# openai/Video-Pre-Training

Hardware: NVIDIA H100
Metric: frames/sec MinecraftPolicy fwd, 128x128x3 BxT=128x128 (higher is better)
Workload: dtype bf16

## Files before the change

video-pre-training_b200/csrc/common.cuh:

```cuda
#pragma once
#include <cuda.h>
#include <cuda_bf16.h>
#include <cuda_runtime.h>
#include <stdint.h>

#include "../../include/vpt_b200.h"

namespace vpt {

void set_error(const char* fmt, ...);
#define VPT_CHECK(cond, ...)                 \
    do {                                     \
        if (!(cond)) {                       \
            vpt::set_error(__VA_ARGS__);     \
            return VPT_ERR_ARG;              \
        }                                    \
    } while (0)
#define VPT_CUDA(expr)                                                                   \
    do {                                                                                 \
        cudaError_t _e = (expr);                                                         \
        if (_e != cudaSuccess) {                                                         \
            vpt::set_error("%s failed: %s (%s:%d)", #expr, cudaGetErrorString(_e), __FILE__, __LINE__); \
            return VPT_ERR_CUDA;                                                         \
        }                                                                                \
    } while (0)
#define VPT_LAUNCH_CHECK() VPT_CUDA(cudaGetLastError())
static int g_pdl = 0;
template <typename... KArgs, typename... Args>
static inline void launch_k(void (*kernel)(KArgs...), dim3 grid, dim3 block, size_t smem, cudaStream_t stream, Args&&... args) {
    cudaLaunchConfig_t cfg;
    memset(&cfg, 0, sizeof(cfg));
    cfg.gridDim = grid;
    cfg.blockDim = block;
    cfg.dynamicSmemBytes = smem;
    cfg.stream = stream;
    cudaLaunchAttribute attr[1];
    attr[0].id = cudaLaunchAttributeProgrammaticStreamSerialization;
    attr[0].val.programmaticStreamSerializationAllowed = 1;
    cfg.attrs = attr;
    cfg.numAttrs = g_pdl ? 1 : 0;
    (void)cudaLaunchKernelEx(&cfg, kernel, static_cast<KArgs>(args)...);
}


#ifndef VPT_NO_WATCHDOG
__device__ unsigned int g_device_error = 0;
#endif

__device__ __forceinline__ void pdl_sync() {
    asm volatile("griddepcontrol.launch_dependents;" ::: "memory");
    asm volatile("griddepcontrol.wait;" ::: "memory");
}
__device__ __forceinline__ uint32_t smem_u32(const void* p) { return (uint32_t)__cvta_generic_to_shared(p); }
__device__ __forceinline__ int lane_id() { return threadIdx.x & 31; }

__device__ __forceinline__ float warp_sum(float v) {
#pragma unroll
    for (int o = 16; o > 0; o >>= 1) v += __shfl_xor_sync(0xffffffffu, v, o);
    return v;
}
__device__ __forceinline__ float warp_max(float v) {
#pragma unroll
    for (int o = 16; o > 0; o >>= 1) v = fmaxf(v, __shfl_xor_sync(0xffffffffu, v, o));
    return v;
}

__device__ __forceinline__ uint32_t pack_bf16(float lo, float hi) {
    __nv_bfloat162 v = __floats2bfloat162_rn(lo, hi);
    return *reinterpret_cast<uint32_t*>(&v);
}
__device__ __forceinline__ float bf16_lo(uint32_t v) { return __uint_as_float(v << 16); }
__device__ __forceinline__ float bf16_hi(uint32_t v) { return __uint_as_float(v & 0xffff0000u); }
__device__ __forceinline__ float round_bf16(float v) { return __bfloat162float(__float2bfloat16_rn(v)); }

__device__ __forceinline__ void mbar_init(uint64_t* bar, uint32_t count) {
    asm volatile("mbarrier.init.shared::cta.b64 [%0], %1;" ::"r"(smem_u32(bar)), "r"(count));
}
__device__ __forceinline__ void fence_barrier_init() { asm volatile("fence.mbarrier_init.release.cluster;" ::: "memory"); }
__device__ __forceinline__ void fence_proxy_async() { asm volatile("fence.proxy.async.shared::cta;" ::: "memory"); }
__device__ __forceinline__ void mbar_expect_tx(uint64_t* bar, uint32_t bytes) {
    asm volatile("mbarrier.arrive.expect_tx.shared::cta.b64 _, [%0], %1;" ::"r"(smem_u32(bar)), "r"(bytes) : "memory");
}
__device__ __forceinline__ void mbar_arrive(uint64_t* bar) {
    asm volatile("mbarrier.arrive.shared::cta.b64 _, [%0];" ::"r"(smem_u32(bar)) : "memory");
}
__device__ __forceinline__ bool mbar_try_wait(uint64_t* bar, uint32_t parity) {
    uint32_t ok;
    asm volatile(
        "{\n\t.reg .pred p;\n\t"
        "mbarrier.try_wait.parity.shared::cta.b64 p, [%1], %2;\n\t"
        "selp.b32 %0, 1, 0, p;\n\t}"
        : "=r"(ok)
        : "r"(smem_u32(bar)), "r"(parity)
        : "memory");
    return ok != 0;
}
__device__ __forceinline__ bool mbar_try_wait_sleep(uint64_t* bar, uint32_t parity, uint32_t ns) {
    uint32_t ok;
    asm volatile(
        "{\n\t.reg .pred p;\n\t"
        "mbarrier.try_wait.parity.shared::cta.b64 p, [%1], %2, %3;\n\t"
        "selp.b32 %0, 1, 0, p;\n\t}"
        : "=r"(ok)
        : "r"(smem_u32(bar)), "r"(parity), "r"(ns)
        : "memory");
    return ok != 0;
}
__device__ __forceinline__ bool mbar_wait(uint64_t* bar, uint32_t parity, unsigned int code) {
    if (mbar_try_wait(bar, parity)) return true;
    const long long t0 = clock64();
    for (unsigned int it = 1;; ++it) {
        if (mbar_try_wait_sleep(bar, parity, 20000u)) return true;
        if ((it & 63u) == 0u) {
            if (*(volatile unsigned int*)&g_device_error != 0u) return false;
            if (clock64() - t0 > 3000000000LL) {
                atomicCAS(&g_device_error, 0u, code);
                return false;
            }
        }
    }
}

__device__ __forceinline__ void tma_prefetch_desc(const CUtensorMap* m) {
    asm volatile("prefetch.tensormap [%0];" ::"l"((uint64_t)m) : "memory");
}
__device__ __forceinline__ void tma_load_2d(void* dst, const CUtensorMap* m, uint64_t* bar, int c0, int c1) {
    asm volatile(
        "cp.async.bulk.tensor.2d.shared::cluster.global.tile.mbarrier::complete_tx::bytes [%0], [%1, {%3, %4}], [%2];" ::"r"(
            smem_u32(dst)),
        "l"((uint64_t)m), "r"(smem_u32(bar)), "r"(c0), "r"(c1)
        : "memory");
}
__device__ __forceinline__ void tma_load_4d(void* dst, const CUtensorMap* m, uint64_t* bar, int c0, int c1, int c2, int c3) {
    asm volatile(
        "cp.async.bulk.tensor.4d.shared::cluster.global.tile.mbarrier::complete_tx::bytes [%0], [%1, {%3, %4, %5, %6}], [%2];" ::"r"(
            smem_u32(dst)),
        "l"((uint64_t)m), "r"(smem_u32(bar)), "r"(c0), "r"(c1), "r"(c2), "r"(c3)
        : "memory");
}

__device__ __forceinline__ void tma_store_2d(const CUtensorMap* m, const void* src, int c0, int c1) {
    asm volatile("cp.async.bulk.tensor.2d.global.shared::cta.bulk_group [%0, {%2, %3}], [%1];" ::"l"((uint64_t)m), "r"(smem_u32(src)), "r"(c0),
                 "r"(c1)
                 : "memory");
}
__device__ __forceinline__ void bulk_commit() { asm volatile("cp.async.bulk.commit_group;" ::: "memory"); }
template <int N>
__device__ __forceinline__ void bulk_wait_read() {
    asm volatile("cp.async.bulk.wait_group.read %0;" ::"n"(N) : "memory");
}
template <int N>
__device__ __forceinline__ void bulk_wait_all() {
    asm volatile("cp.async.bulk.wait_group %0;" ::"n"(N) : "memory");
}
__device__ __forceinline__ void named_bar_sync(int id, int nthreads) { asm volatile("bar.sync %0, %1;" ::"r"(id), "r"(nthreads) : "memory"); }
__device__ __forceinline__ void named_bar_arrive(int id, int nthreads) { asm volatile("bar.arrive %0, %1;" ::"r"(id), "r"(nthreads) : "memory"); }

__device__ __forceinline__ void tma_load_2d_mc(void* dst, const CUtensorMap* m, uint64_t* bar, int c0, int c1, uint16_t cta_mask) {
    asm volatile(
        "cp.async.bulk.tensor.2d.shared::cluster.global.tile.mbarrier::complete_tx::bytes.multicast::cluster [%0], [%1, {%3, %4}], [%2], %5;" ::"r"(
            smem_u32(dst)),
        "l"((uint64_t)m), "r"(smem_u32(bar)), "r"(c0), "r"(c1), "h"(cta_mask)
        : "memory");
}

__device__ __forceinline__ void mbar_arrive_cluster(uint64_t* bar, uint32_t rank) {
    asm volatile(
        "{\n\t.reg .b32 ra;\n\t"
        "mapa.shared::cluster.u32 ra, %0, %1;\n\t"
        "mbarrier.arrive.release.cluster.shared::cluster.b64 _, [ra];\n\t}" ::"r"(smem_u32(bar)),
        "r"(rank)
        : "memory");
}
__device__ __forceinline__ uint32_t cluster_ctarank() {
    uint32_t r;
    asm volatile("mov.u32 %0, %%cluster_ctarank;" : "=r"(r));
    return r;
}
__device__ __forceinline__ void cluster_sync_all() {
    asm volatile("barrier.cluster.arrive.release.aligned;\n\tbarrier.cluster.wait.acquire.aligned;" ::: "memory");
}

__device__ __forceinline__ void wgmma_fence() { asm volatile("wgmma.fence.sync.aligned;" ::: "memory"); }
__device__ __forceinline__ void wgmma_commit() { asm volatile("wgmma.commit_group.sync.aligned;" ::: "memory"); }
template <int N>
__device__ __forceinline__ void wgmma_wait() { asm volatile("wgmma.wait_group.sync.aligned %0;" ::"n"(N) : "memory"); }
template <int N>
__device__ __forceinline__ void wgmma_reg_fence(float (&d)[N]) {
#pragma unroll
    for (int i = 0; i < N; ++i) asm volatile("" : "+f"(d[i])::"memory");
}

template <int TA, int TB>
__device__ __forceinline__ void wgmma_n64(float (&d)[32], uint64_t a_desc, uint64_t b_desc, uint32_t accumulate) {
    asm volatile(
        "{\n\t.reg .pred p;\n\t"
        "setp.ne.b32 p, %34, 0;\n\t"
        "wgmma.mma_async.sync.aligned.m64n64k16.f32.bf16.bf16 "
        "{%0, %1, %2, %3, %4, %5, %6, %7, %8, %9, %10, %11, %12, %13, %14, %15, %16, %17, %18, %19, %20, %21, %22, %23, %24, %25, %26, %27, %28, %29, %30, %31}, %32, %33, p, 1, 1, %35, %36;\n\t}"
        : "+f"(d[0]), "+f"(d[1]), "+f"(d[2]), "+f"(d[3]), "+f"(d[4]), "+f"(d[5]), "+f"(d[6]), "+f"(d[7]), "+f"(d[8]), "+f"(d[9]), "+f"(d[10]), "+f"(d[11]), "+f"(d[12]), "+f"(d[13]), "+f"(d[14]), "+f"(d[15]), "+f"(d[16]), "+f"(d[17]), "+f"(d[18]), "+f"(d[19]), "+f"(d[20]), "+f"(d[21]), "+f"(d[22]), "+f"(d[23]), "+f"(d[24]), "+f"(d[25]), "+f"(d[26]), "+f"(d[27]), "+f"(d[28]), "+f"(d[29]), "+f"(d[30]), "+f"(d[31])
        : "l"(a_desc), "l"(b_desc), "r"(accumulate), "n"(TA), "n"(TB)
        : "memory");
}

template <int TA, int TB>
__device__ __forceinline__ void wgmma_n128(float (&d)[64], uint64_t a_desc, uint64_t b_desc, uint32_t accumulate) {
    asm volatile(
        "{\n\t.reg .pred p;\n\t"
        "setp.ne.b32 p, %66, 0;\n\t"
        "wgmma.mma_async.sync.aligned.m64n128k16.f32.bf16.bf16 "
        "{%0, %1, %2, %3, %4, %5, %6, %7, %8, %9, %10, %11, %12, %13, %14, %15, %16, %17, %18, %19, %20, %21, %22, %23, %24, %25, %26, %27, %28, %29, %30, %31, %32, %33, %34, %35, %36, %37, %38, %39, %40, %41, %42, %43, %44, %45, %46, %47, %48, %49, %50, %51, %52, %53, %54, %55, %56, %57, %58, %59, %60, %61, %62, %63}, %64, %65, p, 1, 1, %67, %68;\n\t}"
        : "+f"(d[0]), "+f"(d[1]), "+f"(d[2]), "+f"(d[3]), "+f"(d[4]), "+f"(d[5]), "+f"(d[6]), "+f"(d[7]), "+f"(d[8]), "+f"(d[9]), "+f"(d[10]), "+f"(d[11]), "+f"(d[12]), "+f"(d[13]), "+f"(d[14]), "+f"(d[15]), "+f"(d[16]), "+f"(d[17]), "+f"(d[18]), "+f"(d[19]), "+f"(d[20]), "+f"(d[21]), "+f"(d[22]), "+f"(d[23]), "+f"(d[24]), "+f"(d[25]), "+f"(d[26]), "+f"(d[27]), "+f"(d[28]), "+f"(d[29]), "+f"(d[30]), "+f"(d[31]), "+f"(d[32]), "+f"(d[33]), "+f"(d[34]), "+f"(d[35]), "+f"(d[36]), "+f"(d[37]), "+f"(d[38]), "+f"(d[39]), "+f"(d[40]), "+f"(d[41]), "+f"(d[42]), "+f"(d[43]), "+f"(d[44]), "+f"(d[45]), "+f"(d[46]), "+f"(d[47]), "+f"(d[48]), "+f"(d[49]), "+f"(d[50]), "+f"(d[51]), "+f"(d[52]), "+f"(d[53]), "+f"(d[54]), "+f"(d[55]), "+f"(d[56]), "+f"(d[57]), "+f"(d[58]), "+f"(d[59]), "+f"(d[60]), "+f"(d[61]), "+f"(d[62]), "+f"(d[63])
        : "l"(a_desc), "l"(b_desc), "r"(accumulate), "n"(TA), "n"(TB)
        : "memory");
}

template <int R>
__device__ __forceinline__ void setmaxnreg_dec() { asm volatile("setmaxnreg.dec.sync.aligned.u32 %0;" ::"n"(R)); }
template <int R>
__device__ __forceinline__ void setmaxnreg_inc() { asm volatile("setmaxnreg.inc.sync.aligned.u32 %0;" ::"n"(R)); }

__device__ __forceinline__ uint64_t gmma_desc_sw128(uint32_t smem_addr, uint32_t lbo_bytes = 16u, uint32_t sbo_bytes = 1024u) {
    uint64_t d = 0;
    d |= (uint64_t)((smem_addr & 0x3FFFFu) >> 4);
    d |= (uint64_t)(lbo_bytes >> 4) << 16;
    d |= (uint64_t)(sbo_bytes >> 4) << 32;
    d |= (uint64_t)1 << 62;
    return d;
}

template <int NR>
__device__ __forceinline__ void wgmma_frag_store(const float (&d)[NR], float* stg, int pitch, int col0) {
    const int w = (threadIdx.x >> 5) & 3, l = threadIdx.x & 31;
    const int r0 = 16 * w + (l >> 2), c0 = col0 + 2 * (l & 3);
#pragma unroll
    for (int i = 0; i < NR / 4; ++i) {
        *reinterpret_cast<float2*>(stg + (size_t)r0 * pitch + c0 + 8 * i) = make_float2(d[4 * i], d[4 * i + 1]);
        *reinterpret_cast<float2*>(stg + (size_t)(r0 + 8) * pitch + c0 + 8 * i) = make_float2(d[4 * i + 2], d[4 * i + 3]);
    }
}
template <int C, int NR>
__device__ __forceinline__ void wgmma_frag_store_chunk(const float (&d)[NR], float* blk, int pitch) {
    static_assert(16 * C + 16 <= NR, "chunk outside the fragment");
    const int l = threadIdx.x & 31;
    float* dst = blk + (size_t)(l >> 2) * pitch + 2 * (l & 3);
#pragma unroll
    for (int i = 0; i < 4; ++i) {
        *reinterpret_cast<float2*>(dst + 8 * i) = make_float2(d[16 * C + 4 * i], d[16 * C + 4 * i + 1]);
        *reinterpret_cast<float2*>(dst + (size_t)8 * pitch + 8 * i) = make_float2(d[16 * C + 4 * i + 2], d[16 * C + 4 * i + 3]);
    }
}
__device__ __forceinline__ void stg_ld_32(const float* src, uint32_t (&v)[32]) {
#pragma unroll
    for (int q = 0; q < 8; ++q) {
        const float4 x = reinterpret_cast<const float4*>(src)[q];
        v[4 * q] = __float_as_uint(x.x); v[4 * q + 1] = __float_as_uint(x.y); v[4 * q + 2] = __float_as_uint(x.z); v[4 * q + 3] = __float_as_uint(x.w);
    }
}

}
```

video-pre-training_b200/csrc/firstconv.cuh:

```cuda
#pragma once
#include <type_traits>

#include "attention.cuh"
#include "common.cuh"

namespace vpt {

constexpr int kFcTile = 8;
constexpr int kFcConv = 2 * kFcTile + 1;
constexpr int kFcIn = kFcConv + 2;
constexpr int kFcThreads = 256;
constexpr int kFcPos = kFcConv * kFcConv;
constexpr int kFcMTiles = (kFcPos + 15) / 16;
constexpr int kFcPatchElems = kFcIn * kFcIn * 3;
constexpr int kFcPatchBytes = 2192;

template <typename TIN>
struct FcIn {
    static constexpr bool kF32 = std::is_same<TIN, float>::value;
    static constexpr int kKSteps = kF32 ? 6 : 4;
    static constexpr int kBPitch = 16 * kKSteps + 8;
    static constexpr int kPatches = kF32 ? 2 : 1;
};

template <bool F32OUT, typename TIN>
__global__ void __launch_bounds__(kFcThreads, 2) firstconv_pool_kernel(const TIN* __restrict__ img, const float* __restrict__ w,
                                                                       const float* __restrict__ bias, void* __restrict__ out_,
                                                                       float2* __restrict__ stat_part, int H, int W, int C0, long long total_tiles, int zp) {
    pdl_sync();
    extern __shared__ __align__(16) uint8_t fc_smem[];
    using In = FcIn<TIN>;
    constexpr int kBPitch = In::kBPitch, kKCols = 16 * In::kKSteps;
    __nv_bfloat16* patch = reinterpret_cast<__nv_bfloat16*>(fc_smem);
    __nv_bfloat16* patch_lo = reinterpret_cast<__nv_bfloat16*>(fc_smem + kFcPatchBytes);
    __nv_bfloat16* Bs = reinterpret_cast<__nv_bfloat16*>(fc_smem + In::kPatches * kFcPatchBytes);
    using CT = typename std::conditional<F32OUT, float, __nv_bfloat16>::type;
    const int CB = F32OUT ? 64 : C0;
    const int cpitch = CB + 8;
    CT* ctile = reinterpret_cast<CT*>(Bs + (size_t)C0 * kBPitch);
    CT* const out = reinterpret_cast<CT*>(out_);
    const int tiles_x = (W / 2) / kFcTile, tiles_y = (H / 2) / kFcTile;
    const int tiles = tiles_x * tiles_y;

    for (int i = threadIdx.x; i < C0 * kKCols; i += kFcThreads) {
        const int n = i / kKCols, k = i % kKCols;
        float v = 0.f;
        if (k >= 64) {
            if (k < 64 + 27) v = __ldg(w + n * 27 + k - 64);
        } else if (k < 27) {
            v = __ldg(w + n * 27 + k);
        } else if (k < 54) {
            const float x = __ldg(w + n * 27 + k - 27);
            v = x - __bfloat162float(__float2bfloat16_rn(x));
        } else if (k == 54) {
            v = __ldg(bias + n);
        } else if (k == 55) {
            const float x = __ldg(bias + n);
            v = x - __bfloat162float(__float2bfloat16_rn(x));
        }
        Bs[n * kBPitch + k] = __float2bfloat16_rn(v);
    }

    const int warp = threadIdx.x >> 5, lane = threadIdx.x & 31, g = lane >> 2, tg = lane & 3;
    int koff[4][4];
    bool kval[4][4];
#pragma unroll
    for (int s = 0; s < 4; ++s)
#pragma unroll
        for (int e = 0; e < 4; ++e) {
            const int k = 16 * s + 2 * tg + (e & 1) + ((e >> 1) << 3);
            const int kk = k < 27 ? k : k - 27;
            kval[s][e] = k < 54;
            koff[s][e] = kval[s][e] ? (kk / 9) * (kFcIn * 3) + kk % 9 : 0;
        }

    constexpr int kPE = (kFcPatchElems + kFcThreads - 1) / kFcThreads;
    int pe_row[kPE], pe_col[kPE];
#pragma unroll
    for (int j = 0; j < kPE; ++j) {
        const int i = threadIdx.x + j * kFcThreads;
        pe_row[j] = i / (kFcIn * 3);
        pe_col[j] = i % (kFcIn * 3);
    }
    TIN pre[kPE];
    auto prefetch = [&](long long tid) {
        const long long f = tid / tiles;
        const int tile = (int)(tid % tiles);
        const int Yin0 = 2 * (tile / tiles_x) * kFcTile - 2, Xin0 = 2 * (tile % tiles_x) * kFcTile - 2;
        const TIN* fimg = img + f * (long long)H * W * 3;
#pragma unroll
        for (int j = 0; j < kPE; ++j) {
            const int Y = Yin0 + pe_row[j], xb = Xin0 * 3 + pe_col[j];
            const bool ok = (threadIdx.x + j * kFcThreads < kFcPatchElems) && Y >= 0 && Y < H && xb >= 0 && xb < W * 3;
            pre[j] = ok ? __ldg(fimg + (long long)Y * W * 3 + xb) : (TIN)0;
        }
    };
    if ((long long)blockIdx.x < total_tiles) prefetch(blockIdx.x);

  for (long long tid = blockIdx.x; tid < total_tiles; tid += gridDim.x) {
    const long long f = tid / tiles;
    const int tile = (int)(tid % tiles);
    const int PY0 = (tile / tiles_x) * kFcTile, PX0 = (tile % tiles_x) * kFcTile;
    int any_lo = 0;
    if constexpr (In::kF32) {
        int nz = 0;
#pragma unroll
        for (int j = 0; j < kPE; ++j) {
            const int i = threadIdx.x + j * kFcThreads;
            if (i < kFcPatchElems) {
                const __nv_bfloat16 hi = __float2bfloat16_rn(pre[j]);
                const float lo = pre[j] - __bfloat162float(hi);
                patch[i] = hi;
                patch_lo[i] = __float2bfloat16_rn(lo);
                nz |= lo != 0.f;
            }
        }
        any_lo = __syncthreads_or(nz);
    } else {
#pragma unroll
        for (int j = 0; j < kPE; ++j) {
            const int i = threadIdx.x + j * kFcThreads;
            if (i < kFcPatchElems) patch[i] = __float2bfloat16_rn((float)pre[j]);
        }
    }
    if (tid + gridDim.x < total_tiles) prefetch(tid + gridDim.x);
    const int Ho = H / 2, Wo = W / 2, opitch = Wo + zp;
    CT* fout = out + f * (long long)(Ho + zp) * opitch * C0;
  for (int cg = 0; cg < C0; cg += CB) {
    __syncthreads();

    for (int mt = warp; mt < kFcMTiles; mt += kFcThreads / 32) {
        int pos[2], pbase[2];
        bool inimg[2];
#pragma unroll
        for (int rr = 0; rr < 2; ++rr) {
            const int p = min(mt * 16 + g + rr * 8, kFcPos - 1);
            pos[rr] = mt * 16 + g + rr * 8;
            const int cy = p / kFcConv, cx = p % kFcConv;
            pbase[rr] = (cy * kFcIn + cx) * 3;
            const int Y = 2 * PY0 - 1 + cy, X = 2 * PX0 - 1 + cx;
            inimg[rr] = (Y >= 0 && Y < H && X >= 0 && X < W);
        }
        uint32_t af[4][4];
#pragma unroll
        for (int s = 0; s < 4; ++s) {
#pragma unroll
            for (int rr = 0; rr < 2; ++rr) {
#pragma unroll
                for (int hh = 0; hh < 2; ++hh) {
                    const uint16_t lo = kval[s][2 * hh] ? *reinterpret_cast<const uint16_t*>(patch + pbase[rr] + koff[s][2 * hh]) : (uint16_t)0;
                    const uint16_t hi = kval[s][2 * hh + 1] ? *reinterpret_cast<const uint16_t*>(patch + pbase[rr] + koff[s][2 * hh + 1]) : (uint16_t)0;
                    af[s][rr + 2 * hh] = (uint32_t)lo | ((uint32_t)hi << 16);
                }
            }
        }
        if (tg == 3) af[3][0] = af[3][1] = 0x3F803F80u;

        for (int nh = cg / 64; nh < (cg + CB) / 64; ++nh) {
            float acc[8][4];
#pragma unroll
            for (int nt = 0; nt < 8; ++nt) acc[nt][0] = acc[nt][1] = acc[nt][2] = acc[nt][3] = 0.f;
#pragma unroll
            for (int s = 0; s < 4; ++s) {
#pragma unroll
                for (int np = 0; np < 4; ++np) {
                    uint32_t b0, b1, b2, b3;
                    const int nrow = nh * 64 + np * 16 + (lane & 7) + ((lane >> 4) << 3);
                    const int kcol = s * 16 + (((lane >> 3) & 1) << 3);
                    ldsm_x4(smem_u32(Bs + nrow * kBPitch + kcol), b0, b1, b2, b3);
                    mma_bf16_16816(acc[2 * np], af[s][0], af[s][1], af[s][2], af[s][3], b0, b1);
                    mma_bf16_16816(acc[2 * np + 1], af[s][0], af[s][1], af[s][2], af[s][3], b2, b3);
                }
            }
            if constexpr (In::kF32) {
                if (any_lo) {
#pragma unroll
                    for (int s = 0; s < 2; ++s) {
                        uint32_t af_lo[4];
#pragma unroll
                        for (int rr = 0; rr < 2; ++rr)
#pragma unroll
                            for (int hh = 0; hh < 2; ++hh) {
                                const int k = 16 * s + 2 * tg + 8 * hh;
                                const uint16_t lo = k < 27 ? *reinterpret_cast<const uint16_t*>(patch_lo + pbase[rr] + koff[s][2 * hh]) : (uint16_t)0;
                                const uint16_t hi = k + 1 < 27 ? *reinterpret_cast<const uint16_t*>(patch_lo + pbase[rr] + koff[s][2 * hh + 1]) : (uint16_t)0;
                                af_lo[rr + 2 * hh] = (uint32_t)lo | ((uint32_t)hi << 16);
                            }
#pragma unroll
                        for (int np = 0; np < 4; ++np) {
                            uint32_t b0, b1, b2, b3;
                            const int nrow = nh * 64 + np * 16 + (lane & 7) + ((lane >> 4) << 3);
                            const int kcol = 64 + s * 16 + (((lane >> 3) & 1) << 3);
                            ldsm_x4(smem_u32(Bs + nrow * kBPitch + kcol), b0, b1, b2, b3);
                            mma_bf16_16816(acc[2 * np], af_lo[0], af_lo[1], af_lo[2], af_lo[3], b0, b1);
                            mma_bf16_16816(acc[2 * np + 1], af_lo[0], af_lo[1], af_lo[2], af_lo[3], b2, b3);
                        }
                    }
                }
            }
#pragma unroll
            for (int rr = 0; rr < 2; ++rr) {
                if (pos[rr] >= kFcPos) continue;
                CT* crow = ctile + (size_t)pos[rr] * cpitch + (nh * 64 - cg) + 2 * tg;
#pragma unroll
                for (int nt = 0; nt < 8; ++nt) {
                    const float v0 = inimg[rr] ? acc[nt][2 * rr] : 0.f;
                    const float v1 = inimg[rr] ? acc[nt][2 * rr + 1] : 0.f;
                    if constexpr (F32OUT) *reinterpret_cast<float2*>(crow + nt * 8) = make_float2(v0, v1);
                    else *reinterpret_cast<uint32_t*>(crow + nt * 8) = pack_bf16(v0, v1);
                }
            }
        }
    }
    __syncthreads();

    if constexpr (F32OUT) {
        const int C4 = CB / 4;
        for (int i = threadIdx.x; i < kFcTile * kFcTile * C4; i += kFcThreads) {
            const int c4 = i % C4, px = (i / C4) % kFcTile, py = i / (C4 * kFcTile);
            float4 m = make_float4(0.f, 0.f, 0.f, 0.f);
#pragma unroll
            for (int dy = 0; dy < 3; ++dy)
#pragma unroll
                for (int dx = 0; dx < 3; ++dx) {
                    const int p = (2 * py + dy) * kFcConv + 2 * px + dx;
                    const float4 v = *reinterpret_cast<const float4*>(ctile + (size_t)p * cpitch + 4 * c4);
                    m.x = fmaxf(m.x, v.x); m.y = fmaxf(m.y, v.y); m.z = fmaxf(m.z, v.z); m.w = fmaxf(m.w, v.w);
                }
            *reinterpret_cast<float4*>(fout + ((long long)(PY0 + py) * opitch + PX0 + px) * C0 + cg + 4 * c4) = m;
        }
    } else {
    const int C8 = C0 / 8;
    for (int i = threadIdx.x; i < kFcTile * kFcTile * C8; i += kFcThreads) {
        const int c8 = i % C8, px = (i / C8) % kFcTile, py = i / (C8 * kFcTile);
        uint4 m = make_uint4(0, 0, 0, 0);
#pragma unroll
        for (int dy = 0; dy < 3; ++dy)
#pragma unroll
            for (int dx = 0; dx < 3; ++dx) {
                const int p = (2 * py + dy) * kFcConv + 2 * px + dx;
                const uint4 v = *reinterpret_cast<const uint4*>(ctile + (size_t)p * cpitch + 8 * c8);
                m.x = bf16x2_max(m.x, v.x); m.y = bf16x2_max(m.y, v.y);
                m.z = bf16x2_max(m.z, v.z); m.w = bf16x2_max(m.w, v.w);
            }
        *reinterpret_cast<uint4*>(fout + ((long long)(PY0 + py) * opitch + PX0 + px) * C0 + 8 * c8) = m;
    }
    }
  }
    if (zp) {
        const int C8 = C0 * (int)sizeof(CT) / 16;
        uint4* fo = reinterpret_cast<uint4*>(fout);
        const bool right = (PX0 + kFcTile == Wo), bottom = (PY0 + kFcTile == Ho);
        if (right)
            for (int i = threadIdx.x; i < kFcTile * C8; i += kFcThreads)
                fo[((long long)(PY0 + i / C8) * opitch + Wo) * C8 + (i % C8)] = make_uint4(0, 0, 0, 0);
        if (bottom)
            for (int i = threadIdx.x; i < (kFcTile + (right ? 1 : 0)) * C8; i += kFcThreads)
                fo[((long long)Ho * opitch + PX0 + i / C8) * C8 + (i % C8)] = make_uint4(0, 0, 0, 0);
    }
    __syncthreads();
    if (stat_part) {
        for (int c = threadIdx.x; c < C0; c += kFcThreads) {
            float cs = 0.f, css = 0.f;
            for (int py = 0; py < kFcTile; ++py)
                for (int px = 0; px < kFcTile; ++px) {
                    const CT o = fout[((long long)(PY0 + py) * opitch + PX0 + px) * C0 + c];
                    float v;
                    if constexpr (F32OUT) v = o;
                    else v = __bfloat162float(o);
                    cs += v;
                    css = fmaf(v, v, css);
                }
            stat_part[(f * tiles + tile) * C0 + c] = make_float2(cs, css);
        }
    }
  }
}

}

extern "C" int vpt_firstconv_stat_parts(int32_t F, int32_t H, int32_t W, int32_t C0) {
    (void)F;
    return (H / 16) * (W / 16) * C0;
}

extern "C" int vpt_set_firstconv_mode(int32_t mode) {
    (void)mode;
    return VPT_OK;
}

namespace vpt {

template <typename TIN>
static int firstconv_pool_launch(const char* fn, const TIN* img, const float* w, const float* bias, void* out, float* stat_part, int32_t F,
                                 int32_t H, int32_t W, int32_t C0, int32_t zp, int32_t out_f32, void* stream) {
    VPT_CHECK(img && w && bias && out && F > 0, "%s: null argument", fn);
    VPT_CHECK(H % 16 == 0 && W % 16 == 0 && H >= 16 && W >= 16, "%s: H, W must be multiples of 16 (H=%d W=%d)", fn, H, W);
    VPT_CHECK(C0 == 64 || C0 == 128 || C0 == 192 || C0 == 256, "%s: C0=%d not in {64,128,192,256}", fn, C0);
    const long long blocks = (long long)F * (H / 16) * (W / 16);
    VPT_CHECK(blocks < 2147483647LL, "%s: too many tiles", fn);
    using In = FcIn<TIN>;
    const int CB = out_f32 ? 64 : C0;
    const size_t smem = (size_t)In::kPatches * kFcPatchBytes + (size_t)C0 * In::kBPitch * 2 + (size_t)kFcPos * (CB + 8) * (out_f32 ? 4 : 2);
    void (*kern)(const TIN*, const float*, const float*, void*, float2*, int, int, int, long long, int) =
        out_f32 ? firstconv_pool_kernel<true, TIN> : firstconv_pool_kernel<false, TIN>;
    static size_t attr[2] = {0, 0};
    if (smem > attr[out_f32 ? 1 : 0]) {
        VPT_CUDA(cudaFuncSetAttribute(kern, cudaFuncAttributeMaxDynamicSharedMemorySize, (int)smem));
        attr[out_f32 ? 1 : 0] = smem;
    }
    int per_sm = (int)((227 * 1024) / (smem + 1024));
    if (per_sm > 2) per_sm = 2;
    if (per_sm < 1) per_sm = 1;
    long long grid = (long long)num_sms() * per_sm;
    if (grid > blocks) grid = blocks;
    launch_k(kern, dim3((unsigned)grid), dim3(kFcThreads), smem, (cudaStream_t)stream,
             img, w, bias, out, reinterpret_cast<float2*>(stat_part), H, W, C0, blocks, zp ? 1 : 0);
    VPT_LAUNCH_CHECK();
    return VPT_OK;
}

}

extern "C" int vpt_firstconv_pool(const uint8_t* img, const float* w, const float* bias, void* out, float* stat_part, int32_t F,
                                  int32_t H, int32_t W, int32_t C0, int32_t zp, int32_t out_f32, void* stream) {
    return vpt::firstconv_pool_launch("vpt_firstconv_pool", img, w, bias, out, stat_part, F, H, W, C0, zp, out_f32, stream);
}

extern "C" int vpt_firstconv_pool_f32(const float* img, const float* w, const float* bias, void* out, float* stat_part, int32_t F,
                                      int32_t H, int32_t W, int32_t C0, int32_t zp, int32_t out_f32, void* stream) {
    return vpt::firstconv_pool_launch("vpt_firstconv_pool_f32", img, w, bias, out, stat_part, F, H, W, C0, zp, out_f32, stream);
}
```

Baseline: 27630.

## Port first conv+pool kernel to register-A wgmma with swizzled B and fused stats

Replaces the per-warp mma.sync m16n8k16 loop with warpgroup wgmma (A from registers, B from a 128B-swizzled shared layout) for the first conv, aligning shared memory to 1024 bytes. The max-pool is restructured so each thread produces a 2x2 block of outputs from a 5x5 window, reusing loaded rows. Per-tile channel statistics are computed from pooled values staged in shared memory rather than re-read from global output. This cuts instruction overhead and global re-reads, at the cost of wgmma wait per N chunk and more complex descriptor/swizzle correctness.

Measured after the change: 28040 (median of 6 runs). 1.01x the previous value.

```diff
diff --git a/video-pre-training_b200/csrc/common.cuh b/video-pre-training_b200/csrc/common.cuh
--- a/video-pre-training_b200/csrc/common.cuh
+++ b/video-pre-training_b200/csrc/common.cuh
@@ -215,6 +215,23 @@
         : "memory");
 }
 
+template <int TB>
+__device__ __forceinline__ void wgmma_rs_n64(float (&d)[32], const uint32_t (&a)[4], uint64_t b_desc) {
+    asm volatile(
+        "{\n\t.reg .pred p;\n\t"
+        "setp.ne.b32 p, 1, 0;\n\t"
+        "wgmma.mma_async.sync.aligned.m64n64k16.f32.bf16.bf16 "
+        "{%0, %1, %2, %3, %4, %5, %6, %7, %8, %9, %10, %11, %12, %13, %14, %15, %16, %17, %18, %19, %20, %21, %22, %23, %24, %25, %26, %27, %28, %29, %30, %31}, {%32, %33, %34, %35}, %36, p, 1, 1, %37;\n\t}"
+        : "+f"(d[0]), "+f"(d[1]), "+f"(d[2]), "+f"(d[3]), "+f"(d[4]), "+f"(d[5]), "+f"(d[6]), "+f"(d[7]), "+f"(d[8]), "+f"(d[9]), "+f"(d[10]), "+f"(d[11]), "+f"(d[12]), "+f"(d[13]), "+f"(d[14]), "+f"(d[15]), "+f"(d[16]), "+f"(d[17]), "+f"(d[18]), "+f"(d[19]), "+f"(d[20]), "+f"(d[21]), "+f"(d[22]), "+f"(d[23]), "+f"(d[24]), "+f"(d[25]), "+f"(d[26]), "+f"(d[27]), "+f"(d[28]), "+f"(d[29]), "+f"(d[30]), "+f"(d[31])
+        : "r"(a[0]), "r"(a[1]), "r"(a[2]), "r"(a[3]), "l"(b_desc), "n"(TB)
+        : "memory");
+}
+template <int N>
+__device__ __forceinline__ void wgmma_reg_fence(uint32_t (&r)[N]) {
+#pragma unroll
+    for (int i = 0; i < N; ++i) asm volatile("" : "+r"(r[i])::"memory");
+}
+
 template <int R>
 __device__ __forceinline__ void setmaxnreg_dec() { asm volatile("setmaxnreg.dec.sync.aligned.u32 %0;" ::"n"(R)); }
 template <int R>
diff --git a/video-pre-training_b200/csrc/firstconv.cuh b/video-pre-training_b200/csrc/firstconv.cuh
--- a/video-pre-training_b200/csrc/firstconv.cuh
+++ b/video-pre-training_b200/csrc/firstconv.cuh
@@ -1,8 +1,8 @@
 #pragma once
 #include <type_traits>
 
-#include "attention.cuh"
 #include "common.cuh"
+#include "elementwise.cuh"
 
 namespace vpt {
 
@@ -11,43 +11,56 @@
 constexpr int kFcIn = kFcConv + 2;
 constexpr int kFcThreads = 256;
 constexpr int kFcPos = kFcConv * kFcConv;
-constexpr int kFcMTiles = (kFcPos + 15) / 16;
+constexpr int kFcMBlocks = (kFcPos + 63) / 64;
 constexpr int kFcPatchElems = kFcIn * kFcIn * 3;
 constexpr int kFcPatchBytes = 2192;
+constexpr int kFcN = 64;
 
 template <typename TIN>
 struct FcIn {
     static constexpr bool kF32 = std::is_same<TIN, float>::value;
-    static constexpr int kKSteps = kF32 ? 6 : 4;
-    static constexpr int kBPitch = 16 * kKSteps + 8;
     static constexpr int kPatches = kF32 ? 2 : 1;
 };
+
+static inline size_t firstconv_smem(int C0, bool f32_in, bool out_f32) {
+    const int CB = out_f32 ? 64 : C0;
+    return 1024 + (size_t)C0 * 128 + (f32_in ? 2 : 1) * (size_t)kFcPatchBytes + (size_t)kFcPos * (CB + 8) * (out_f32 ? 4 : 2);
+}
+
+template <typename CT>
+__device__ __forceinline__ uint4 fc_max16(uint4 a, uint4 b) {
+    if constexpr (std::is_same<CT, float>::value) {
+        return make_uint4(__float_as_uint(fmaxf(__uint_as_float(a.x), __uint_as_float(b.x))), __float_as_uint(fmaxf(__uint_as_float(a.y), __uint_as_float(b.y))),
+                          __float_as_uint(fmaxf(__uint_as_float(a.z), __uint_as_float(b.z))), __float_as_uint(fmaxf(__uint_as_float(a.w), __uint_as_float(b.w))));
+    } else {
+        return make_uint4(bf16x2_max(a.x, b.x), bf16x2_max(a.y, b.y), bf16x2_max(a.z, b.z), bf16x2_max(a.w, b.w));
+    }
+}
 
 template <bool F32OUT, typename TIN>
 __global__ void __launch_bounds__(kFcThreads, 2) firstconv_pool_kernel(const TIN* __restrict__ img, const float* __restrict__ w,
                                                                        const float* __restrict__ bias, void* __restrict__ out_,
                                                                        float2* __restrict__ stat_part, int H, int W, int C0, long long total_tiles, int zp) {
     pdl_sync();
-    extern __shared__ __align__(16) uint8_t fc_smem[];
+    extern __shared__ uint8_t fc_smem_raw[];
+    const uint32_t raw = smem_u32(fc_smem_raw);
+    uint8_t* fc_smem = fc_smem_raw + (((raw + 1023u) & ~1023u) - raw);
     using In = FcIn<TIN>;
-    constexpr int kBPitch = In::kBPitch, kKCols = 16 * In::kKSteps;
-    __nv_bfloat16* patch = reinterpret_cast<__nv_bfloat16*>(fc_smem);
-    __nv_bfloat16* patch_lo = reinterpret_cast<__nv_bfloat16*>(fc_smem + kFcPatchBytes);
-    __nv_bfloat16* Bs = reinterpret_cast<__nv_bfloat16*>(fc_smem + In::kPatches * kFcPatchBytes);
+    __nv_bfloat16* Bs = reinterpret_cast<__nv_bfloat16*>(fc_smem);
+    __nv_bfloat16* patch = reinterpret_cast<__nv_bfloat16*>(fc_smem + (size_t)C0 * 128);
+    __nv_bfloat16* patch_lo = patch + kFcPatchBytes / 2;
     using CT = typename std::conditional<F32OUT, float, __nv_bfloat16>::type;
     const int CB = F32OUT ? 64 : C0;
     const int cpitch = CB + 8;
-    CT* ctile = reinterpret_cast<CT*>(Bs + (size_t)C0 * kBPitch);
+    CT* ctile = reinterpret_cast<CT*>(fc_smem + (size_t)C0 * 128 + In::kPatches * kFcPatchBytes);
     CT* const out = reinterpret_cast<CT*>(out_);
     const int tiles_x = (W / 2) / kFcTile, tiles_y = (H / 2) / kFcTile;
     const int tiles = tiles_x * tiles_y;
 
-    for (int i = threadIdx.x; i < C0 * kKCols; i += kFcThreads) {
-        const int n = i / kKCols, k = i % kKCols;
+    for (int i = threadIdx.x; i < C0 * 64; i += kFcThreads) {
+        const int n = i >> 6, k = i & 63;
         float v = 0.f;
-        if (k >= 64) {
-            if (k < 64 + 27) v = __ldg(w + n * 27 + k - 64);
-        } else if (k < 27) {
+        if (k < 27) {
             v = __ldg(w + n * 27 + k);
         } else if (k < 54) {
             const float x = __ldg(w + n * 27 + k - 27);
@@ -58,48 +71,44 @@
             const float x = __ldg(bias + n);
             v = x - __bfloat162float(__float2bfloat16_rn(x));
         }
-        Bs[n * kBPitch + k] = __float2bfloat16_rn(v);
-    }
-
-    const int warp = threadIdx.x >> 5, lane = threadIdx.x & 31, g = lane >> 2, tg = lane & 3;
-    int koff[4][4];
-    bool kval[4][4];
-#pragma unroll
-    for (int s = 0; s < 4; ++s)
+        Bs[n * 64 + ((((k >> 3) ^ (n & 7)) << 3) | (k & 7))] = __float2bfloat16_rn(v);
+    }
+    fence_proxy_async();
+    const uint32_t b_base = smem_u32(Bs);
+
+    const int warp = threadIdx.x >> 5, wg = threadIdx.x >> 7, lane = threadIdx.x & 31, g = lane >> 2, tg = lane & 3;
+    uint32_t koff8[4];
+#pragma unroll
+    for (int s = 0; s < 4; ++s) {
+        koff8[s] = 0;
 #pragma unroll
         for (int e = 0; e < 4; ++e) {
             const int k = 16 * s + 2 * tg + (e & 1) + ((e >> 1) << 3);
             const int kk = k < 27 ? k : k - 27;
-            kval[s][e] = k < 54;
-            koff[s][e] = kval[s][e] ? (kk / 9) * (kFcIn * 3) + kk % 9 : 0;
-        }
+            koff8[s] |= (uint32_t)(k < 54 ? (kk / 9) * (kFcIn * 3) + kk % 9 : 0) << (8 * e);
+        }
+    }
+    auto koff = [&](int s, int e) { return (int)((koff8[s] >> (8 * e)) & 0xFFu); };
 
     constexpr int kPE = (kFcPatchElems + kFcThreads - 1) / kFcThreads;
-    int pe_row[kPE], pe_col[kPE];
-#pragma unroll
-    for (int j = 0; j < kPE; ++j) {
-        const int i = threadIdx.x + j * kFcThreads;
-        pe_row[j] = i / (kFcIn * 3);
-        pe_col[j] = i % (kFcIn * 3);
-    }
     TIN pre[kPE];
-    auto prefetch = [&](long long tid) {
-        const long long f = tid / tiles;
-        const int tile = (int)(tid % tiles);
+    const int ntiles = (int)total_tiles;
+    auto prefetch = [&](int tid) {
+        const int f = tid / tiles, tile = tid % tiles;
         const int Yin0 = 2 * (tile / tiles_x) * kFcTile - 2, Xin0 = 2 * (tile % tiles_x) * kFcTile - 2;
-        const TIN* fimg = img + f * (long long)H * W * 3;
+        const TIN* fimg = img + (long long)f * H * W * 3;
 #pragma unroll
         for (int j = 0; j < kPE; ++j) {
-            const int Y = Yin0 + pe_row[j], xb = Xin0 * 3 + pe_col[j];
-            const bool ok = (threadIdx.x + j * kFcThreads < kFcPatchElems) && Y >= 0 && Y < H && xb >= 0 && xb < W * 3;
+            const int i = threadIdx.x + j * kFcThreads;
+            const int Y = Yin0 + i / (kFcIn * 3), xb = Xin0 * 3 + i % (kFcIn * 3);
+            const bool ok = (i < kFcPatchElems) && Y >= 0 && Y < H && xb >= 0 && xb < W * 3;
             pre[j] = ok ? __ldg(fimg + (long long)Y * W * 3 + xb) : (TIN)0;
         }
     };
-    if ((long long)blockIdx.x < total_tiles) prefetch(blockIdx.x);
-
-  for (long long tid = blockIdx.x; tid < total_tiles; tid += gridDim.x) {
-    const long long f = tid / tiles;
-    const int tile = (int)(tid % tiles);
+    if ((int)blockIdx.x < ntiles) prefetch(blockIdx.x);
+
+  for (int tid = blockIdx.x; tid < ntiles; tid += gridDim.x) {
+    const int f = tid / tiles, tile = tid % tiles;
     const int PY0 = (tile / tiles_x) * kFcTile, PX0 = (tile % tiles_x) * kFcTile;
     int any_lo = 0;
     if constexpr (In::kF32) {
@@ -123,13 +132,14 @@
             if (i < kFcPatchElems) patch[i] = __float2bfloat16_rn((float)pre[j]);
         }
     }
-    if (tid + gridDim.x < total_tiles) prefetch(tid + gridDim.x);
+    if (tid + (int)gridDim.x < ntiles) prefetch(tid + gridDim.x);
     const int Ho = H / 2, Wo = W / 2, opitch = Wo + zp;
-    CT* fout = out + f * (long long)(Ho + zp) * opitch * C0;
+    CT* fout = out + (long long)f * (Ho + zp) * opitch * C0;
   for (int cg = 0; cg < C0; cg += CB) {
     __syncthreads();
 
-    for (int mt = warp; mt < kFcMTiles; mt += kFcThreads / 32) {
+    for (int mb = wg; mb < kFcMBlocks; mb += 2) {
+        const int mt = 4 * mb + (warp & 3);
         int pos[2], pbase[2];
         bool inimg[2];
 #pragma unroll
@@ -141,110 +151,140 @@
             const int Y = 2 * PY0 - 1 + cy, X = 2 * PX0 - 1 + cx;
             inimg[rr] = (Y >= 0 && Y < H && X >= 0 && X < W);
         }
+        auto ld2 = [&](const __nv_bfloat16* src, int rr, int s, int hh) {
+            const uint32_t lo = *reinterpret_cast<const uint16_t*>(src + pbase[rr] + koff(s, 2 * hh));
+            const uint32_t hi = *reinterpret_cast<const uint16_t*>(src + pbase[rr] + koff(s, 2 * hh + 1));
+            return lo | (hi << 16);
+        };
         uint32_t af[4][4];
 #pragma unroll
-        for (int s = 0; s < 4; ++s) {
-#pragma unroll
-            for (int rr = 0; rr < 2; ++rr) {
-#pragma unroll
-                for (int hh = 0; hh < 2; ++hh) {
-                    const uint16_t lo = kval[s][2 * hh] ? *reinterpret_cast<const uint16_t*>(patch + pbase[rr] + koff[s][2 * hh]) : (uint16_t)0;
-                    const uint16_t hi = kval[s][2 * hh + 1] ? *reinterpret_cast<const uint16_t*>(patch + pbase[rr] + koff[s][2 * hh + 1]) : (uint16_t)0;
-                    af[s][rr + 2 * hh] = (uint32_t)lo | ((uint32_t)hi << 16);
-                }
-            }
-        }
-        if (tg == 3) af[3][0] = af[3][1] = 0x3F803F80u;
-
-        for (int nh = cg / 64; nh < (cg + CB) / 64; ++nh) {
-            float acc[8][4];
-#pragma unroll
-            for (int nt = 0; nt < 8; ++nt) acc[nt][0] = acc[nt][1] = acc[nt][2] = acc[nt][3] = 0.f;
-#pragma unroll
-            for (int s = 0; s < 4; ++s) {
-#pragma unroll
-                for (int np = 0; np < 4; ++np) {
-                    uint32_t b0, b1, b2, b3;
-                    const int nrow = nh * 64 + np * 16 + (lane & 7) + ((lane >> 4) << 3);
-                    const int kcol = s * 16 + (((lane >> 3) & 1) << 3);
-                    ldsm_x4(smem_u32(Bs + nrow * kBPitch + kcol), b0, b1, b2, b3);
-                    mma_bf16_16816(acc[2 * np], af[s][0], af[s][1], af[s][2], af[s][3], b0, b1);
-                    mma_bf16_16816(acc[2 * np + 1], af[s][0], af[s][1], af[s][2], af[s][3], b2, b3);
-                }
-            }
+        for (int s = 0; s < 3; ++s)
+#pragma unroll
+            for (int rr = 0; rr < 2; ++rr)
+#pragma unroll
+                for (int hh = 0; hh < 2; ++hh) af[s][rr + 2 * hh] = ld2(patch, rr, s, hh);
+#pragma unroll
+        for (int rr = 0; rr < 2; ++rr) {
+            af[3][rr] = tg < 3 ? ld2(patch, rr, 3, 0) : 0x3F803F80u;
+            af[3][rr + 2] = 0u;
+        }
+        uint32_t al[In::kF32 ? 2 : 1][4];
+        if constexpr (In::kF32) {
+#pragma unroll
+            for (int s = 0; s < 2; ++s)
+#pragma unroll
+                for (int rr = 0; rr < 2; ++rr)
+#pragma unroll
+                    for (int hh = 0; hh < 2; ++hh) {
+                        const int k = 16 * s + 2 * tg + 8 * hh;
+                        uint32_t lo = 0, hi = 0;
+                        if (any_lo) {
+                            if (k < 27) lo = *reinterpret_cast<const uint16_t*>(patch_lo + pbase[rr] + koff(s, 2 * hh));
+                            if (k + 1 < 27) hi = *reinterpret_cast<const uint16_t*>(patch_lo + pbase[rr] + koff(s, 2 * hh + 1));
+                        }
+                        al[s][rr + 2 * hh] = lo | (hi << 16);
+                    }
+        }
+
+        for (int n0 = cg; n0 < cg + CB; n0 += kFcN) {
+            float acc[kFcN / 2];
+#pragma unroll
+            for (int i = 0; i < kFcN / 2; ++i) acc[i] = 0.f;
+            wgmma_fence();
+#pragma unroll
+            for (int s = 0; s < 4; ++s) wgmma_rs_n64<0>(acc, af[s], gmma_desc_sw128(b_base + n0 * 128 + s * 32));
             if constexpr (In::kF32) {
                 if (any_lo) {
 #pragma unroll
-                    for (int s = 0; s < 2; ++s) {
-                        uint32_t af_lo[4];
-#pragma unroll
-                        for (int rr = 0; rr < 2; ++rr)
-#pragma unroll
-                            for (int hh = 0; hh < 2; ++hh) {
-                                const int k = 16 * s + 2 * tg + 8 * hh;
-                                const uint16_t lo = k < 27 ? *reinterpret_cast<const uint16_t*>(patch_lo + pbase[rr] + koff[s][2 * hh]) : (uint16_t)0;
-                                const uint16_t hi = k + 1 < 27 ? *reinterpret_cast<const uint16_t*>(patch_lo + pbase[rr] + koff[s][2 * hh + 1]) : (uint16_t)0;
-                                af_lo[rr + 2 * hh] = (uint32_t)lo | ((uint32_t)hi << 16);
-                            }
-#pragma unroll
-                        for (int np = 0; np < 4; ++np) {
-                            uint32_t b0, b1, b2, b3;
-                            const int nrow = nh * 64 + np * 16 + (lane & 7) + ((lane >> 4) << 3);
-                            const int kcol = 64 + s * 16 + (((lane >> 3) & 1) << 3);
-                            ldsm_x4(smem_u32(Bs + nrow * kBPitch + kcol), b0, b1, b2, b3);
-                            mma_bf16_16816(acc[2 * np], af_lo[0], af_lo[1], af_lo[2], af_lo[3], b0, b1);
-                            mma_bf16_16816(acc[2 * np + 1], af_lo[0], af_lo[1], af_lo[2], af_lo[3], b2, b3);
-                        }
-                    }
+                    for (int s = 0; s < 2; ++s) wgmma_rs_n64<0>(acc, al[s], gmma_desc_sw128(b_base + n0 * 128 + s * 32));
                 }
             }
+            wgmma_commit();
+            wgmma_wait<0>();
+            wgmma_reg_fence(acc);
 #pragma unroll
             for (int rr = 0; rr < 2; ++rr) {
                 if (pos[rr] >= kFcPos) continue;
-                CT* crow = ctile + (size_t)pos[rr] * cpitch + (nh * 64 - cg) + 2 * tg;
-#pragma unroll
-                for (int nt = 0; nt < 8; ++nt) {
-                    const float v0 = inimg[rr] ? acc[nt][2 * rr] : 0.f;
-                    const float v1 = inimg[rr] ? acc[nt][2 * rr + 1] : 0.f;
+                CT* crow = ctile + (size_t)pos[rr] * cpitch + (n0 - cg) + 2 * tg;
+#pragma unroll
+                for (int nt = 0; nt < kFcN / 8; ++nt) {
+                    const float v0 = inimg[rr] ? acc[4 * nt + 2 * rr] : 0.f;
+                    const float v1 = inimg[rr] ? acc[4 * nt + 2 * rr + 1] : 0.f;
                     if constexpr (F32OUT) *reinterpret_cast<float2*>(crow + nt * 8) = make_float2(v0, v1);
                     else *reinterpret_cast<uint32_t*>(crow + nt * 8) = pack_bf16(v0, v1);
                 }
             }
         }
+#pragma unroll
+        for (int s = 0; s < 4; ++s) wgmma_reg_fence(af[s]);
+        if constexpr (In::kF32) {
+#pragma unroll
+            for (int s = 0; s < 2; ++s) wgmma_reg_fence(al[s]);
+        }
     }
     __syncthreads();
 
-    if constexpr (F32OUT) {
-        const int C4 = CB / 4;
-        for (int i = threadIdx.x; i < kFcTile * kFcTile * C4; i += kFcThreads) {
-            const int c4 = i % C4, px = (i / C4) % kFcTile, py = i / (C4 * kFcTile);
-            float4 m = make_float4(0.f, 0.f, 0.f, 0.f);
-#pragma unroll
-            for (int dy = 0; dy < 3; ++dy)
-#pragma unroll
-                for (int dx = 0; dx < 3; ++dx) {
-                    const int p = (2 * py + dy) * kFcConv + 2 * px + dx;
-                    const float4 v = *reinterpret_cast<const float4*>(ctile + (size_t)p * cpitch + 4 * c4);
-                    m.x = fmaxf(m.x, v.x); m.y = fmaxf(m.y, v.y); m.z = fmaxf(m.z, v.z); m.w = fmaxf(m.w, v.w);
+    const int CV = CB * (int)sizeof(CT) / 16;
+    const int items = (kFcTile / 2) * (kFcTile / 2) * CV;
+    constexpr int kItems = F32OUT ? 1 : 2;
+    uint4 pooled[kItems][4];
+#pragma unroll
+    for (int j = 0; j < kItems; ++j) {
+        const int i = threadIdx.x + j * kFcThreads;
+        if (i < items) {
+            const int cv = i % CV, pq = (i / CV) % (kFcTile / 2), pp = i / (CV * (kFcTile / 2));
+            const CT* src = ctile + (size_t)(4 * pp * kFcConv + 4 * pq) * cpitch + cv * (16 / (int)sizeof(CT));
+            uint4 m[2][2];
+#pragma unroll
+            for (int a = 0; a < 4; ++a) m[a >> 1][a & 1] = make_uint4(0, 0, 0, 0);
+#pragma unroll
+            for (int r = 0; r < 5; ++r) {
+                uint4 v[5];
+#pragma unroll
+                for (int c = 0; c < 5; ++c) v[c] = *reinterpret_cast<const uint4*>(src + (size_t)(r * kFcConv + c) * cpitch);
+                const uint4 h0 = fc_max16<CT>(fc_max16<CT>(v[0], v[1]), v[2]), h1 = fc_max16<CT>(fc_max16<CT>(v[2], v[3]), v[4]);
+                if (r <= 2) {
+                    m[0][0] = fc_max16<CT>(m[0][0], h0);
+                    m[0][1] = fc_max16<CT>(m[0][1], h1);
                 }
-            *reinterpret_cast<float4*>(fout + ((long long)(PY0 + py) * opitch + PX0 + px) * C0 + cg + 4 * c4) = m;
-        }
-    } else {
-    const int C8 = C0 / 8;
-    for (int i = threadIdx.x; i < kFcTile * kFcTile * C8; i += kFcThreads) {
-        const int c8 = i % C8, px = (i / C8) % kFcTile, py = i / (C8 * kFcTile);
-        uint4 m = make_uint4(0, 0, 0, 0);
-#pragma unroll
-        for (int dy = 0; dy < 3; ++dy)
-#pragma unroll
-            for (int dx = 0; dx < 3; ++dx) {
-                const int p = (2 * py + dy) * kFcConv + 2 * px + dx;
-                const uint4 v = *reinterpret_cast<const uint4*>(ctile + (size_t)p * cpitch + 8 * c8);
-                m.x = bf16x2_max(m.x, v.x); m.y = bf16x2_max(m.y, v.y);
-                m.z = bf16x2_max(m.z, v.z); m.w = bf16x2_max(m.w, v.w);
-            }
-        *reinterpret_cast<uint4*>(fout + ((long long)(PY0 + py) * opitch + PX0 + px) * C0 + 8 * c8) = m;
-    }
+                if (r >= 2) {
+                    m[1][0] = fc_max16<CT>(m[1][0], h0);
+                    m[1][1] = fc_max16<CT>(m[1][1], h1);
+                }
+            }
+#pragma unroll
+            for (int a = 0; a < 4; ++a) {
+                const int py = 2 * pp + (a >> 1), px = 2 * pq + (a & 1);
+                *reinterpret_cast<uint4*>(fout + ((long long)(PY0 + py) * opitch + PX0 + px) * C0 + cg + cv * (16 / (int)sizeof(CT))) = m[a >> 1][a & 1];
+                pooled[j][a] = m[a >> 1][a & 1];
+            }
+        }
+    }
+    if (stat_part) {
+        __syncthreads();
+#pragma unroll
+        for (int j = 0; j < kItems; ++j) {
+            const int i = threadIdx.x + j * kFcThreads;
+            if (i < items) {
+                const int cv = i % CV, pq = (i / CV) % (kFcTile / 2), pp = i / (CV * (kFcTile / 2));
+#pragma unroll
+                for (int a = 0; a < 4; ++a)
+                    reinterpret_cast<uint4*>(ctile)[((2 * pp + (a >> 1)) * kFcTile + 2 * pq + (a & 1)) * CV + cv] = pooled[j][a];
+            }
+        }
+        __syncthreads();
+        for (int c = threadIdx.x; c < CB; c += kFcThreads) {
+            float cs = 0.f, css = 0.f;
+#pragma unroll 8
+            for (int q = 0; q < kFcTile * kFcTile; ++q) {
+                float v;
+                if constexpr (F32OUT) v = ctile[q * CB + c];
+                else v = __bfloat162float(ctile[q * CB + c]);
+                cs += v;
+                css = fmaf(v, v, css);
+            }
+            stat_part[(long long)tid * C0 + cg + c] = make_float2(cs, css);
+        }
     }
   }
     if (zp) {
@@ -258,22 +298,6 @@
             for (int i = threadIdx.x; i < (kFcTile + (right ? 1 : 0)) * C8; i += kFcThreads)
                 fo[((long long)Ho * opitch + PX0 + i / C8) * C8 + (i % C8)] = make_uint4(0, 0, 0, 0);
     }
-    __syncthreads();
-    if (stat_part) {
-        for (int c = threadIdx.x; c < C0; c += kFcThreads) {
-            float cs = 0.f, css = 0.f;
-            for (int py = 0; py < kFcTile; ++py)
-                for (int px = 0; px < kFcTile; ++px) {
-                    const CT o = fout[((long long)(PY0 + py) * opitch + PX0 + px) * C0 + c];
-                    float v;
-                    if constexpr (F32OUT) v = o;
-                    else v = __bfloat162float(o);
-                    cs += v;
-                    css = fmaf(v, v, css);
-                }
-            stat_part[(f * tiles + tile) * C0 + c] = make_float2(cs, css);
-        }
-    }
   }
 }
 
@@ -299,9 +323,7 @@
     VPT_CHECK(C0 == 64 || C0 == 128 || C0 == 192 || C0 == 256, "%s: C0=%d not in {64,128,192,256}", fn, C0);
     const long long blocks = (long long)F * (H / 16) * (W / 16);
     VPT_CHECK(blocks < 2147483647LL, "%s: too many tiles", fn);
-    using In = FcIn<TIN>;
-    const int CB = out_f32 ? 64 : C0;
-    const size_t smem = (size_t)In::kPatches * kFcPatchBytes + (size_t)C0 * In::kBPitch * 2 + (size_t)kFcPos * (CB + 8) * (out_f32 ? 4 : 2);
+    const size_t smem = firstconv_smem(C0, FcIn<TIN>::kF32, out_f32 != 0);
     void (*kern)(const TIN*, const float*, const float*, void*, float2*, int, int, int, long long, int) =
         out_f32 ? firstconv_pool_kernel<true, TIN> : firstconv_pool_kernel<false, TIN>;
     static size_t attr[2] = {0, 0};
```
